# dernasherbrezon/sdr-server

Hardware: AMD Instinct MI355X
Metric: input IQ Msamples/s processed (all clients), 2.016 Msps->48 kHz xlating FIR (higher is better)
Workload: dtype f32; 1 GPU; 1024 clients x 48 kHz off one 2.016 Msps cu8 stream, D=42, 505 taps, 262144-byte blocks (BASELINE configs[3]; N=1: the >=1000-client single-GPU target); clients_total=1024, clients_per_gpu=1024, blocks_per_call=8, mode=optimized, parallelism=single GPU, rccl_ranks=1, feed=xlating_multi (C host)

## Files before the change

### sdr-server_amd/csrc/xl_kernels.hip

```cpp
#include "xl_dev_inline.h"

#include <hip/hip_ext.h>

#include <stdlib.h>

__global__ __launch_bounds__(64) void xl_nco_table_kernel(const XlNcoClient *__restrict__ cl, uint32_t n,
                                                          const float2 *state_in, float2 *state_out,
                                                          float2 *__restrict__ tab, const XlPos pos,
                                                          const uint32_t explicit_K, const uint32_t prio,
                                                          const uint32_t lanes) {
  if (prio == 3) __builtin_amdgcn_s_setprio(3);
  else if (prio == 2) __builtin_amdgcn_s_setprio(2);
  else if (prio == 1) __builtin_amdgcn_s_setprio(1);
  if (threadIdx.x >= lanes) return;
  const uint32_t c = blockIdx.x * lanes + threadIdx.x;
  if (c >= n) return;
  const XlNcoClient k = cl[c];
  const XlBnd bnd = xl_nco_bnd(k, pos, explicit_K);
  asm volatile("" ::: "v255", "a255");
  xl_nco_client_chain<true>(k, bnd, 0u, bnd.K, state_in, state_out, tab);
}

#define XLC_RING 64u
XL_DEV uint32_t xl_lds_off(const void *p) { return (uint32_t)(uintptr_t)(__attribute__((address_space(3))) const char *)p; }
XL_DEV void xl_lds_post(const uint32_t addr, const uint32_t v) { asm volatile("ds_write_b32 %0, %1" ::"v"(addr), "v"(v) : "memory"); }
XL_DEV void xl_lds_post64(const uint32_t addr, const v2f v) { asm volatile("ds_write_b64 %0, %1" ::"v"(addr), "v"(v) : "memory"); }
XL_DEV uint32_t xl_lds_poll(const uint32_t addr) {
  uint32_t v;
  asm volatile("ds_read_b32 %0, %1\n\ts_waitcnt lgkmcnt(0)" : "=v"(v) : "v"(addr) : "memory");
  return v;
}

#define XLC_ALIGN ".p2align 6\n\t"
#define XLC_MUL "v_pk_mul_f32 %[t1], %[p], %[inc] op_sel_hi:[1,0]\n\tv_pk_mul_f32 %[t2], %[p], %[inc] op_sel:[0,1] op_sel_hi:[1,1]\n\t"
#define XLC_ADD "v_pk_add_f32 %[p], %[t1], %[t2] op_sel:[0,1] op_sel_hi:[1,0] neg_lo:[0,1]\n\t"
#define XLC_STEP XLC_MUL XLC_ADD
#define XLC_ENTRY                                                       \
  XLC_MUL "ds_write_b64 %[addr], %[p]\n\t" XLC_ADD                      \
  XLC_MUL "v_add_u32 %[cnt], 1, %[cnt]\n\t" XLC_ADD                     \
  XLC_MUL "ds_write_b32 %[paddr], %[cnt]\n\t" XLC_ADD                   \
  XLC_MUL "v_add_u32 %[off], 0x200, %[off]\n\t" XLC_ADD                 \
  XLC_MUL "v_and_b32 %[off], 0x7fff, %[off]\n\t" XLC_ADD                \
  XLC_MUL "v_add_u32 %[addr], %[off], %[base]\n\t" XLC_ADD              \
  XLC_STEP XLC_STEP XLC_STEP XLC_STEP XLC_STEP XLC_STEP XLC_STEP XLC_STEP XLC_STEP XLC_STEP
#define XLC_STEPS10 XLC_STEP XLC_STEP XLC_STEP XLC_STEP XLC_STEP XLC_STEP XLC_STEP XLC_STEP XLC_STEP XLC_STEP
#define XLC_QENTRY(OFFS) XLC_MUL "ds_write_b64 %[addr], %[p] offset:" OFFS "\n\t" XLC_ADD XLC_STEP XLC_STEP
#define XLC_BLOCK_END(N, ADV)                                           \
  XLC_MUL "v_add_u32 %[cnt], " N ", %[cnt]\n\t" XLC_ADD                 \
  XLC_MUL "ds_write_b32 %[paddr], %[cnt]\n\t" XLC_ADD                   \
  XLC_MUL "v_add_u32 %[off], " ADV ", %[off]\n\t" XLC_ADD               \
  XLC_MUL "v_and_b32 %[off], 0x7fff, %[off]\n\t" XLC_ADD                \
  XLC_MUL "v_add_u32 %[addr], %[off], %[base]\n\t" XLC_ADD XLC_STEP XLC_STEP XLC_STEP XLC_STEP XLC_STEP XLC_STEP XLC_STEP XLC_STEP XLC_STEP XLC_STEP
#define XLC_QUAD                                                        \
  XLC_QENTRY("0") XLC_STEP XLC_STEP XLC_STEP XLC_STEPS10                \
  XLC_QENTRY("512") XLC_STEP XLC_STEP XLC_STEP XLC_STEPS10              \
  XLC_QENTRY("1024") XLC_STEP XLC_STEP XLC_STEP XLC_STEPS10             \
  XLC_MUL "ds_write_b64 %[addr], %[p] offset:1536\n\t" XLC_ADD XLC_BLOCK_END("4", "0x800")
#define XLC_E(OFFS) XLC_QENTRY(OFFS) XLC_STEP XLC_STEP XLC_STEP XLC_STEPS10
#define XLC_E7(B0, B1, B2, B3, B4, B5, B6) XLC_E(B0) XLC_E(B1) XLC_E(B2) XLC_E(B3) XLC_E(B4) XLC_E(B5) XLC_E(B6)
#define XLC_E8(B0, B1, B2, B3, B4, B5, B6, B7) XLC_E7(B0, B1, B2, B3, B4, B5, B6) XLC_E(B7)
#define XLC_OCT                                                         \
  XLC_E7("0", "512", "1024", "1536", "2048", "2560", "3072")           \
  XLC_MUL "ds_write_b64 %[addr], %[p] offset:3584\n\t" XLC_ADD XLC_BLOCK_END("8", "0x1000")
#define XLC_HEX                                                         \
  XLC_E8("0", "512", "1024", "1536", "2048", "2560", "3072", "3584")   \
  XLC_E7("4096", "4608", "5120", "5632", "6144", "6656", "7168")       \
  XLC_MUL "ds_write_b64 %[addr], %[p] offset:7680\n\t" XLC_ADD XLC_BLOCK_END("16", "0x2000")
#define XLC_B32                                                         \
  XLC_E8("0", "512", "1024", "1536", "2048", "2560", "3072", "3584")   \
  XLC_E8("4096", "4608", "5120", "5632", "6144", "6656", "7168", "7680") \
  XLC_E8("8192", "8704", "9216", "9728", "10240", "10752", "11264", "11776") \
  XLC_E7("12288", "12800", "13312", "13824", "14336", "14848", "15360") \
  XLC_MUL "ds_write_b64 %[addr], %[p] offset:15872\n\t" XLC_ADD XLC_BLOCK_END("32", "0x4000")
static_assert(XL_PH_STRIDE == 16u && XLC_RING * 64u * 8u == 0x8000u, "XLC_ENTRY is written for 16 steps per entry and a 32 KB ring");

__global__ __launch_bounds__(256) void xl_nco_chain_kernel(const XlNcoClient *__restrict__ cl, uint32_t n,
                                                           const float2 *state_in, const XlChainCalls calls,
                                                           XlPos pos, unsigned long long *stats) {
  asm volatile("" ::: "v255", "a255");
  const unsigned long long t_entry = stats ? wall_clock64() : 0ull;
  __shared__ v2f ring[XLC_RING][64];
  __shared__ uint32_t s_emax;
  __shared__ uint32_t s_prod;
  __shared__ uint32_t s_next[3];
  const uint32_t w = __builtin_amdgcn_readfirstlane(threadIdx.x >> 6), lane = threadIdx.x & 63u;
  const uint32_t c = blockIdx.x * 64u + lane;
  const bool have = c < n;
  XlNcoClient k;
  k.incr = make_float2(1.0f, 0.0f);
  k.out_off = 0u, k.slot = 0u, k.D = 1u, k.rem0 = 0u;
  if (have) k = cl[c];
  v2f p = {1.0f, 0.0f};
  if (w == 0 && have) p = (v2f){state_in[k.slot].x, state_in[k.slot].y};
  unsigned long long cyc = 0ull, ticks = 0ull, wfirst = 0ull;
  uint32_t entries = 0u;
  for (uint32_t call = 0; call < calls.n; ++call, pos = xl_grid_next(pos)) {
    float2 *const tab = calls.tab[call];
    float2 *const state_out = calls.state_out[call];
    if (call) __syncthreads();
    XlBnd bnd = xl_nco_bnd(k, pos, 0xFFFFFFFFu);
    if (!have) bnd.K = 0u;
    const uint32_t K = bnd.K, E = (K + XL_PH_STRIDE - 1u) >> XL_PH_SHIFT;
    if (threadIdx.x == 0) {
      s_emax = 0u;
      s_prod = 0u;
      s_next[0] = 0u, s_next[1] = 1u, s_next[2] = 2u;
    }
    __syncthreads();
    if (w == 0 && E > 0u) atomicMax(&s_emax, E);
    __syncthreads();
    const uint32_t Emax = s_emax;
    const uint32_t a_prod = xl_lds_off(&s_prod), a_ring0 = xl_lds_off(&ring[0][0]), a_ring = xl_lds_off(&ring[0][lane]);
    v2f *__restrict__ o = reinterpret_cast<v2f *>(tab) + (k.out_off >> XL_PH_SHIFT);
    if (w == 0) {
      __builtin_amdgcn_s_setprio(3);
      const v2f inc = {k.incr.x, k.incr.y};
      uint32_t nb = xl_bnd_next(bnd, 0u);
      const uint32_t a_n0 = xl_lds_off(&s_next[0]), a_n1 = xl_lds_off(&s_next[1]), a_n2 = xl_lds_off(&s_next[2]);
      const unsigned long long c0 = stats ? clock64() : 0ull, w0 = stats ? wall_clock64() : 0ull;
      uint32_t e = 0;
      while (e < Emax) {
        uint32_t ev = (e << XL_PH_SHIFT) < K ? (nb < K ? nb : K) : 0xFFFFFFFFu;
#pragma unroll
        for (int sh = 1; sh < 64; sh <<= 1) {
          const uint32_t other = (uint32_t)__shfl_xor((int)ev, sh);
          ev = other < ev ? other : ev;
        }
        const uint32_t evs = __builtin_amdgcn_readfirstlane(ev);
        uint32_t e_stop = evs == 0u ? 0u : (evs - 1u) >> XL_PH_SHIFT;
        e_stop = e_stop < Emax ? e_stop : Emax;
        if (pos.pad & XL_POS_FMA_STEP) e_stop = e;
        if ((e << XL_PH_SHIFT) < K) {
          uint32_t ee = e;
          while (ee < e_stop) {
            if ((ee & (XLC_RING / 2u - 1u)) == 0u && ee >= XLC_RING) {
              const uint32_t q = (ee - XLC_RING / 2u) >> 1;
              for (uint32_t spin = 0; spin < (1u << 22); ++spin) {
                if (xl_lds_poll(a_n0) >= q && xl_lds_poll(a_n1) >= q && xl_lds_poll(a_n2) >= q) break;
                __builtin_amdgcn_s_sleep(1);
              }
            }
            const uint32_t next_check = (ee | (XLC_RING / 2u - 1u)) + 1u;
            const uint32_t chunk_end = e_stop < next_check ? e_stop : next_check;
            uint32_t off = ((ee & (XLC_RING - 1u)) << 9) + lane * (uint32_t)sizeof(v2f);
            uint32_t addr = a_ring0 + off, cnt = ee;
            v2f t1, t2;
#define XLC_RUN(BLOCK)                                                                                            \
  asm volatile(XLC_ALIGN BLOCK                                                                                   \
               : [p] "+v"(p), [off] "+v"(off), [addr] "+v"(addr), [cnt] "+v"(cnt), [t1] "=&v"(t1), [t2] "=&v"(t2) \
               : [inc] "v"(inc), [base] "v"(a_ring0), [paddr] "v"(a_prod)                                        \
               : "memory")
            for (; ee < chunk_end && (ee & 3u) != 0u; ++ee) XLC_RUN(XLC_ENTRY);
            if ((ee & 7u) == 4u && ee + 4u <= chunk_end) {
              XLC_RUN(XLC_QUAD);
              ee += 4u;
            }
            if ((ee & 15u) == 8u && ee + 8u <= chunk_end) {
              XLC_RUN(XLC_OCT);
              ee += 8u;
            }
            if ((ee & 31u) == 16u && ee + 16u <= chunk_end) {
              XLC_RUN(XLC_HEX);
              ee += 16u;
            }
            for (; ee + 32u <= chunk_end; ee += 32u) XLC_RUN(XLC_B32);
            for (; ee + 16u <= chunk_end; ee += 16u) XLC_RUN(XLC_HEX);
            for (; ee + 8u <= chunk_end; ee += 8u) XLC_RUN(XLC_OCT);
            for (; ee + 4u <= chunk_end; ee += 4u) XLC_RUN(XLC_QUAD);
            for (; ee < chunk_end; ++ee) XLC_RUN(XLC_ENTRY);
#undef XLC_RUN
          }
        }
        if (e_stop > e) e = e_stop;
        if (e < Emax) {
          if ((e & (XLC_RING / 2u - 1u)) == 0u && e >= XLC_RING) {
            const uint32_t q = (e - XLC_RING / 2u) >> 1;
            for (uint32_t spin = 0; spin < (1u << 22); ++spin) {
              if (xl_lds_poll(a_n0) >= q && xl_lds_poll(a_n1) >= q && xl_lds_poll(a_n2) >= q) break;
              __builtin_amdgcn_s_sleep(1);
            }
          }
          const uint32_t m0 = e << XL_PH_SHIFT;
          if (m0 < K) xl_lds_post64(a_ring + (e & (XLC_RING - 1u)) * 64u * (uint32_t)sizeof(v2f), p);
          xl_lds_post(a_prod, e + 1u);
          for (uint32_t m = m0; m < m0 + XL_PH_STRIDE && m < K; ++m) {
            p = xl_nco_next_any(p, inc, bnd.flags);
            if (m + 1u == nb) {
              p = xl_nco_renorm(p);
              nb = xl_bnd_next(bnd, m + 1u);
            }
          }
          ++e;
        }
      }
      if (have) state_out[k.slot] = make_float2(p.x, p.y);
      if (stats) {
        cyc += clock64() - c0;
        const unsigned long long w1 = wall_clock64();
        ticks += w1 - w0;
        entries += Emax;
        if (call == 0u) wfirst = w0;
        if (lane == 0u && blockIdx.x < 1024u) {
          stats[8192u + 8u * blockIdx.x + 1u + 2u * call] = w0 - t_entry;
          stats[8192u + 8u * blockIdx.x + 2u + 2u * call] = w1 - t_entry;
        }
      }
      continue;
    }
    const uint32_t j = w - 1u;
    const uint32_t a_next = xl_lds_off(&s_next[j]);
    v4f *__restrict__ o4 = reinterpret_cast<v4f *>(o);
    for (uint32_t q = j; 2u * q < Emax; q += 3u) {
      const uint32_t need = 2u * q + 2u < Emax ? 2u * q + 2u : Emax;
      for (uint32_t spin = 0; spin < (1u << 24); ++spin) {
        if (xl_lds_poll(a_prod) >= need) break;
        __builtin_amdgcn_s_sleep(1);
      }
      if (2u * q < E) {
        v2f a, b2 = {0.0f, 0.0f};
        const uint32_t ra = a_ring + ((2u * q) & (XLC_RING - 1u)) * 64u * (uint32_t)sizeof(v2f);
        const uint32_t rb = a_ring + ((2u * q + 1u) & (XLC_RING - 1u)) * 64u * (uint32_t)sizeof(v2f);
        const bool two = 2u * q + 1u < E;
        asm volatile("ds_read_b64 %0, %1" : "=v"(a) : "v"(ra) : "memory");
        if (two) asm volatile("ds_read_b64 %0, %1" : "=v"(b2) : "v"(rb) : "memory");
        asm volatile("s_waitcnt lgkmcnt(0)" ::: "memory");
        if (two) o4[q] = (v4f){a.x, a.y, b2.x, b2.y};
        else o[2u * q] = a;
      }
      xl_lds_post(a_next, q + 3u);
    }
    xl_lds_post(a_next, 0xFFFFFFFFu);
  }
  if (stats) __syncthreads();
  if (stats && threadIdx.x == 0u) {
    if (blockIdx.x < 1024u) {
      stats[8192u + 8u * blockIdx.x] = t_entry;
      stats[8192u + 8u * blockIdx.x + 7u] = wall_clock64() - t_entry;
    }
    stats[4u * blockIdx.x] = cyc;
    stats[4u * blockIdx.x + 1u] = ticks;
    stats[4u * blockIdx.x + 2u] = entries;
    stats[4u * blockIdx.x + 3u] = wfirst;
  }
}

template <int FMT>
XL_DEV void xl_stage_window(const XlFirArgs &a, const uint32_t zero_below, const uint32_t win0, const uint32_t wlen,
                            v2f *__restrict__ win) {
  const uint32_t bd = blockDim.x;
  for (uint32_t j0 = threadIdx.x; j0 < wlen; j0 += 4u * bd) {
    v2f v[4];
    bool ok[4];
#pragma unroll
    for (int u = 0; u < 4; ++u) {
      const uint32_t j = j0 + u * bd;
      const uint32_t s = win0 + j;
      const bool first = s < a.n0;
      ok[u] = j < wlen && s >= zero_below && (first || s - a.n0 < a.n1);
      const void *src = (first || !ok[u]) ? a.in0 : a.in1;
      const uint32_t idx = ok[u] ? (first ? s : s - a.n0) : 0u;
      v[u] = xl_sample(src, FMT, idx);
    }
#pragma unroll
    for (int u = 0; u < 4; ++u) {
      const uint32_t j = j0 + u * bd;
      if (j < wlen) win[j] = ok[u] ? v[u] : (v2f){0.0f, 0.0f};
    }
  }
}

template <int CT, int MODE, bool WIDE>
__global__ __launch_bounds__(64 * XL_NW_MAX) __attribute__((amdgpu_num_sgpr(96))) void xl_fir_kernel(const XlFirArgs a) {
  extern __shared__ __attribute__((aligned(16))) v2f xl_win[];
  const uint32_t OT = a.ota;

  if (blockIdx.x < a.nco_blocks) {
    if (((a.flags >> 4) & 3u) == 3u) __builtin_amdgcn_s_setprio(3);
    else if (((a.flags >> 4) & 3u) == 2u) __builtin_amdgcn_s_setprio(2);
    else if (((a.flags >> 4) & 3u) == 1u) __builtin_amdgcn_s_setprio(1);
    const uint32_t nwave = threadIdx.x >> 6, nlane = threadIdx.x & 63u;
    if (nwave < a.nco_wpw && nlane < XL_NCO_LANES) {
      const unsigned long long t0 = a.trace ? wall_clock64() : 0ull;
      const uint32_t c = (blockIdx.x * a.nco_wpw + nwave) * XL_NCO_LANES + nlane;
      if (c < a.nco_nclients) {
        const XlNcoClient k = a.nco_clients[c];
        const XlBnd bnd = xl_nco_bnd(k, xl_grid_next(a.pos), 0xFFFFFFFFu);
        xl_nco_client_chain<false>(k, bnd, 0u, bnd.K, a.nco_state_in, a.nco_state_out, a.nco_tab);
      }
      if (a.trace && nlane == 0) {
        unsigned long long *tn = a.trace + ((size_t)blockIdx.x * XL_NW_MAX + nwave) * 6;
        tn[0] = t0;
        tn[3] = wall_clock64();
        tn[4] = __builtin_amdgcn_s_getreg((4 << 0) | (0 << 6) | (31 << 11));
        tn[5] = __builtin_amdgcn_s_getreg((20 << 0) | (0 << 6) | (31 << 11));
      }
    }
    return;
  }

  if (!(a.flags & 2u)) __builtin_amdgcn_s_setprio(3);
  const uint32_t b = blockIdx.x - a.nco_blocks;
  const unsigned long long t_entry = a.trace ? wall_clock64() : 0ull;

  const uint32_t roll_blocks = gridDim.x - a.nco_blocks < XL_ROLL_BLOCKS ? gridDim.x - a.nco_blocks : XL_ROLL_BLOCKS;
  if (a.hist_out != nullptr && b < roll_blocks) {
    const uint16_t *__restrict__ h0 = reinterpret_cast<const uint16_t *>(a.in0);
    const uint16_t *__restrict__ h1 = reinterpret_cast<const uint16_t *>(a.in1);
    uint16_t *__restrict__ ho = reinterpret_cast<uint16_t *>(a.hist_out);
    const uint32_t hu = a.hist_units, nu = a.block_units;
    for (uint32_t j = b * blockDim.x + threadIdx.x; j < hu; j += roll_blocks * blockDim.x) {
      const uint32_t sidx = nu + j;
      ho[j] = (sidx < hu) ? h0[sidx] : h1[sidx - hu];
    }
  }
  const uint32_t xcd = b & 7u, idx = b >> 3;
  const uint32_t total = a.ngroups * a.xtiles;
  const uint32_t per = total >> 3, extra = total & 7u;
  const uint32_t len = per + (xcd < extra ? 1u : 0u);
  if (idx >= len) return;
  const uint32_t wi = xcd * per + (xcd < extra ? xcd : extra) + idx;
  const uint32_t y = wi / a.xtiles;
  const uint32_t x = wi - y * a.xtiles;
  if (y >= a.ngroups) return;

  const cu32_p g = (cu32_p)(uintptr_t)(a.groups + y);
  const uint32_t D = g[0], Tpad = g[2], ntiles = g[4];
  const XlDyn d = a.explicit_dyn ? a.dyn1 : xl_grid_dyn(D, g[1], g[3], g[7], a.pos);
  const uint32_t K = d.K;
  const bool live = x * OT < K;
  if (!live && a.nco_lanes == 0u) return;

  const uint32_t w = __builtin_amdgcn_readfirstlane(threadIdx.x >> 6);
  v2f phs[CT];
#pragma unroll
  for (int c = 0; c < CT; ++c) phs[c] = (v2f){1.0f, 0.0f};
  if (live) {
    if (w < ntiles) {
      constexpr uint32_t G = 64u / XL_PH_STRIDE;
      const uint32_t lane = threadIdx.x & 63u;
      v2f *__restrict__ pl = xl_win + w * (CT * 64u);
      const uint32_t *__restrict__ tg = reinterpret_cast<const uint32_t *>(a.groups + y) + 8u + w * XL_TILE_DWORDS;
      const uint32_t c = lane / G, e = lane % G;
      const uint32_t m0 = x * OT + e * XL_PH_STRIDE;
      if (c < tg[1] && e * XL_PH_STRIDE < OT && m0 < K) {
        const uint32_t off = tg[2 + c];
        const float2 ci = reinterpret_cast<const float2 *>(tg + 2 + XL_CT_MAX)[c];
        const uint32_t left = K - m0, span = OT < XL_PH_STRIDE ? OT : XL_PH_STRIDE;
        XlBnd bnd;
        bnd.j0 = d.j0, bnd.D = D, bnd.S = a.pos.S, bnd.G = a.explicit_dyn ? 1u : a.pos.G, bnd.K = K, bnd.flags = a.pos.pad;
        v2f *__restrict__ dst = pl + c * 64u + e * XL_PH_STRIDE;
        xl_phase_walk((reinterpret_cast<const v2f *>(a.phtab) + (off >> XL_PH_SHIFT))[m0 >> XL_PH_SHIFT], m0,
                      left < span ? left : span, (v2f){ci.x, ci.y}, bnd, [&](uint32_t i, v2f ph) { dst[i] = ph; });
      }
      __builtin_amdgcn_wave_barrier();
#pragma unroll
      for (int cc = 0; cc < CT; ++cc) phs[cc] = pl[cc * 64u + lane];
    }
    __syncthreads();

    const uint32_t win0 = d.base + x * OT * D;
    const uint32_t wlen = (OT - 1u) * D + Tpad;
    if (a.fmt == XLF_CU8) xl_stage_window<XLF_CU8>(a, d.zero_below, win0, wlen, xl_win);
    else if (a.fmt == XLF_CS8) xl_stage_window<XLF_CS8>(a, d.zero_below, win0, wlen, xl_win);
    else if (a.fmt == XLF_CS16) xl_stage_window<XLF_CS16>(a, d.zero_below, win0, wlen, xl_win);
    else xl_stage_window<XLF_CF32>(a, d.zero_below, win0, wlen, xl_win);
  }
  __syncthreads();

  if (w >= ntiles) {
    const uint32_t nlane = threadIdx.x & 63u;
    const uint32_t slot = (g[6] + (w - ntiles)) * a.xtiles + x;
    if (a.nco_lanes != 0u && slot < a.nco_slots && nlane < a.nco_lanes) {
      __builtin_amdgcn_s_setprio(3);
      const unsigned long long t0 = a.trace ? wall_clock64() : 0ull;
      const uint32_t c = slot * a.nco_lanes + nlane;
      if (c < a.nco_nclients) {
        const XlNcoClient k = a.nco_clients[c];
        const XlBnd bnd = xl_nco_bnd(k, xl_grid_next(a.pos), 0xFFFFFFFFu);
        xl_nco_client_chain<false>(k, bnd, 0u, bnd.K, a.nco_state_in, a.nco_state_out, a.nco_tab);
      }
      if (a.trace && nlane == 0) {
        unsigned long long *tn = a.trace + ((size_t)blockIdx.x * XL_NW_MAX + w) * 6;
        tn[0] = t0;
        tn[3] = wall_clock64();
        tn[4] = __builtin_amdgcn_s_getreg((4 << 0) | (0 << 6) | (31 << 11));
        tn[5] = __builtin_amdgcn_s_getreg((20 << 0) | (0 << 6) | (31 << 11));
      }
    }
    return;
  }
  if (!live) return;
  const uint32_t lane = threadIdx.x & 63u;
  unsigned long long *tr = a.trace ? a.trace + ((size_t)blockIdx.x * XL_NW_MAX + w) * 6 : nullptr;
  if (tr && lane == 0) {
    tr[0] = t_entry;
    tr[1] = wall_clock64();
    tr[4] = __builtin_amdgcn_s_getreg((4 << 0) | (0 << 6) | (31 << 11));
    tr[5] = __builtin_amdgcn_s_getreg((20 << 0) | (0 << 6) | (31 << 11));
  }
  const cu32_p t = g + 8 + w * XL_TILE_DWORDS;
  const uint32_t ncl = t[1];
  const cfloat_p tp = (cfloat_p)(uintptr_t)(a.taps + t[0]);

  XlAcc<MODE> acc[CT];
#pragma unroll
  for (int c = 0; c < CT; ++c) acc[c].clear();

  constexpr int STEP = (CT == 9 || CT == 10) ? 6 : 4;
  const v2f *lp = xl_win + (lane >= OT ? 0u : lane) * D;
#define XL_TAP_LOOP(I0, I1)                                                                       \
  for (uint32_t i = (I0); i < (I1); i += STEP) {                                                  \
    v2f xs[STEP];                                                                                 \
    if (WIDE) {                                                                                   \
      _Pragma("unroll") for (int u = 0; u < STEP; u += 2) {                                       \
        const v4f q = *reinterpret_cast<const v4f *>(lp + i + u);                                 \
        xs[u] = (v2f){q.x, q.y};                                                                  \
        xs[u + 1] = (v2f){q.z, q.w};                                                              \
      }                                                                                           \
    } else {                                                                                      \
      _Pragma("unroll") for (int u = 0; u < STEP; ++u) xs[u] = lp[i + u];                         \
    }                                                                                             \
    const cfloat_p tq = tp + (size_t)i * (2 * CT);                                                \
    _Pragma("unroll") for (int u = 0; u < STEP; ++u) {                                            \
      _Pragma("unroll") for (int c = 0; c < CT; ++c)                                              \
        acc[c].mac(xs[u], tq[(u * CT + c) * 2], tq[(u * CT + c) * 2 + 1]);                        \
    }                                                                                             \
  }
  if (a.flags & 2u) {
    XL_TAP_LOOP(0u, Tpad)
  } else {
    const uint32_t steps = Tpad / STEP;
    const uint32_t b1 = steps / 2, b2 = (7 * steps) / 8;
    const uint32_t e1 = b1 * STEP < Tpad ? b1 * STEP : Tpad;
    const uint32_t e2 = b2 * STEP < Tpad ? b2 * STEP : Tpad;
    __builtin_amdgcn_s_setprio(2);
    XL_TAP_LOOP(0u, e1)
    __builtin_amdgcn_s_setprio(1);
    XL_TAP_LOOP(e1, e2)
    __builtin_amdgcn_s_setprio(0);
    XL_TAP_LOOP(e2, Tpad)
    __builtin_amdgcn_s_setprio(3);
  }
#undef XL_TAP_LOOP

  if (tr && lane == 0) tr[2] = wall_clock64();
  v2f *__restrict__ out = reinterpret_cast<v2f *>(a.out);
  {
    const uint32_t m = x * OT + lane;
    if (m < K && lane < OT) {
#pragma unroll
      for (int c = 0; c < CT; ++c) {
        if ((uint32_t)c < ncl) out[t[2 + c] + m] = xl_rotate<MODE>(acc[c].value(), phs[c]);
      }
    }
  }
  if (tr && lane == 0) {
    __builtin_amdgcn_s_waitcnt(0);
    tr[3] = wall_clock64();
  }
}

size_t xl_fir_lds_bytes_ota(uint32_t D, uint32_t Tpad, uint32_t ota) {
  return ((size_t)(ota - 1u) * D + Tpad) * sizeof(v2f);
}

uint32_t xl_fir_pick_ota(uint32_t D, uint32_t Tpad, size_t budget) {
  for (uint32_t ota = 64; ota >= 8; ota >>= 1)
    if (xl_fir_lds_bytes_ota(D, Tpad, ota) <= budget) return ota;
  return 0;
}

template <int CT, int MODE, bool WIDE>
static hipError_t xl_fir_go2(int nw, const XlFirArgs &a, size_t lds, hipStream_t s) {
  static bool attr_done = false;
  if (!attr_done) {
    hipError_t e = hipFuncSetAttribute(reinterpret_cast<const void *>(&xl_fir_kernel<CT, MODE, WIDE>),
                                       hipFuncAttributeMaxDynamicSharedMemorySize, 160 * 1024);
    if (e != hipSuccess) return e;
    attr_done = true;
  }
  const uint32_t nblocks = a.nco_blocks + 8u * ((a.ngroups * a.xtiles + 7u) / 8u);
  if (nblocks == 0) return hipSuccess;
  const size_t need = (size_t)nw * CT * 64u * sizeof(float2);
  if (lds < need) lds = need;
  hipLaunchKernelGGL((xl_fir_kernel<CT, MODE, WIDE>), dim3(nblocks), dim3(64 * nw), lds, s, a);
  return hipGetLastError();
}

template <int CT, int MODE>
static hipError_t xl_fir_go(int nw, const XlFirArgs &a, size_t lds, hipStream_t s) {
  return (a.flags & 1u) ? xl_fir_go2<CT, MODE, true>(nw, a, lds, s) : xl_fir_go2<CT, MODE, false>(nw, a, lds, s);
}

hipError_t xl_launch_fir(int ct, int mode, int nw, const XlFirArgs &a, size_t lds, hipStream_t s) {
  if (lds > 160 * 1024 || nw < 1 || nw > XL_NW_MAX) return hipErrorInvalidValue;
  if (a.ota != 64 && a.ota != 32 && a.ota != 16 && a.ota != 8) return hipErrorInvalidValue;
  switch (ct * 2 + (mode ? 1 : 0)) {
    case 2: return xl_fir_go<1, 0>(nw, a, lds, s);
    case 3: return xl_fir_go<1, 1>(nw, a, lds, s);
    case 4: return xl_fir_go<2, 0>(nw, a, lds, s);
    case 5: return xl_fir_go<2, 1>(nw, a, lds, s);
    case 8: return xl_fir_go<4, 0>(nw, a, lds, s);
    case 9: return xl_fir_go<4, 1>(nw, a, lds, s);
    case 16: return xl_fir_go<8, 0>(nw, a, lds, s);
    case 17: return xl_fir_go<8, 1>(nw, a, lds, s);
    case 18: return xl_fir_go<9, 0>(nw, a, lds, s);
    case 19: return xl_fir_go<9, 1>(nw, a, lds, s);
    case 20: return xl_fir_go<10, 0>(nw, a, lds, s);
    case 21: return xl_fir_go<10, 1>(nw, a, lds, s);
    case 24: return xl_fir_go<12, 0>(nw, a, lds, s);
    case 25: return xl_fir_go<12, 1>(nw, a, lds, s);
    default: return hipErrorInvalidValue;
  }
}

hipError_t xl_launch_nco_table(const XlNcoClient *clients, uint32_t nclients, const float2 *state_in,
                               float2 *state_out, float2 *phtab, XlPos pos, uint32_t explicit_K, uint32_t prio,
                               hipStream_t s) {
  if (nclients == 0) return hipSuccess;
  const uint32_t lanes = XL_NCO_LANES;
  hipLaunchKernelGGL(xl_nco_table_kernel, dim3((nclients + lanes - 1) / lanes), dim3(64), 0, s, clients, nclients,
                     state_in, state_out, phtab, pos, explicit_K, prio, lanes);
  return hipGetLastError();
}

hipError_t xl_launch_nco_chain(const XlNcoClient *clients, uint32_t nclients, const float2 *state_in,
                               const XlChainCalls &calls, XlPos pos, unsigned long long *stats, hipStream_t s,
                               hipEvent_t done) {
  if (calls.n < 1u || calls.n > XL_CHAIN_MAXCALLS) return hipErrorInvalidValue;
  if (nclients == 0) return done ? hipEventRecord(done, s) : hipSuccess;
  if (done)
    hipExtLaunchKernelGGL(xl_nco_chain_kernel, dim3((nclients + 63u) / 64u), dim3(256), 0, s, nullptr, done, 0, clients,
                          nclients, state_in, calls, pos, stats);
  else
    hipLaunchKernelGGL(xl_nco_chain_kernel, dim3((nclients + 63u) / 64u), dim3(256), 0, s, clients, nclients, state_in,
                       calls, pos, stats);
  return hipGetLastError();
}

__global__ void xl_convert_cf32_kernel(const void *__restrict__ raw, int fmt, uint32_t n, v2f *__restrict__ dst) {
  for (uint32_t i = blockIdx.x * blockDim.x + threadIdx.x; i < n; i += gridDim.x * blockDim.x)
    dst[i] = xl_sample(raw, fmt, i);
}

hipError_t xl_launch_convert_cf32(const void *raw, int fmt, uint32_t nsamples, float2 *dst, hipStream_t s) {
  if (nsamples == 0) return hipSuccess;
  const uint32_t blocks = (nsamples + 255) / 256 < 2048 ? (nsamples + 255) / 256 : 2048;
  hipLaunchKernelGGL(xl_convert_cf32_kernel, dim3(blocks), dim3(256), 0, s, raw, fmt, nsamples,
                     reinterpret_cast<v2f *>(dst));
  return hipGetLastError();
}

__global__ void xl_convert_q15_kernel(const void *__restrict__ raw, int fmt, uint32_t n, int16_t *__restrict__ dst) {
  for (uint32_t i = blockIdx.x * blockDim.x + threadIdx.x; i < n; i += gridDim.x * blockDim.x) {
    int32_t v;
    if (fmt == XLF_CU8) {
      v = ((int32_t) reinterpret_cast<const uint8_t *>(raw)[i] - 128) * 256;
    } else if (fmt == XLF_CS8) {
      v = (int32_t) reinterpret_cast<const int8_t *>(raw)[i] * 256;
    } else {
      v = reinterpret_cast<const int16_t *>(raw)[i];
    }
    dst[i] = (int16_t)v;
  }
}

hipError_t xl_launch_convert_q15(const void *raw, int fmt, uint32_t nelems, int16_t *dst, hipStream_t s) {
  if (nelems == 0) return hipSuccess;
  const uint32_t blocks = (nelems + 255) / 256 < 2048 ? (nelems + 255) / 256 : 2048;
  hipLaunchKernelGGL(xl_convert_q15_kernel, dim3(blocks), dim3(256), 0, s, raw, fmt, nelems, dst);
  return hipGetLastError();
}

__global__ __launch_bounds__(1024) void xl_move_down_kernel(uint32_t *buf, uint32_t from_dw, uint32_t count_dw) {
  for (uint32_t base = 0; base < count_dw; base += 1024) {
    const uint32_t i = base + threadIdx.x;
    uint32_t v = 0;
    if (i < count_dw) v = buf[from_dw + i];
    __syncthreads();
    if (i < count_dw) buf[i] = v;
    __syncthreads();
  }
}

hipError_t xl_launch_move_down(void *buf, uint32_t from, uint32_t count, uint32_t elem_bytes, hipStream_t s) {
  if (count == 0 || from == 0) return hipSuccess;
  const uint32_t k = elem_bytes / 4;
  hipLaunchKernelGGL(xl_move_down_kernel, dim3(1), dim3(1024), 0, s, reinterpret_cast<uint32_t *>(buf), from * k,
                     count * k);
  return hipGetLastError();
}

__global__ void xl_update_history_kernel(const uint16_t *__restrict__ hist, const uint16_t *__restrict__ block,
                                         uint32_t h_u, uint32_t n_u, uint16_t *__restrict__ out) {
  for (uint32_t j = blockIdx.x * blockDim.x + threadIdx.x; j < h_u; j += gridDim.x * blockDim.x) {
    const uint32_t s = n_u + j;
    out[j] = (s < h_u) ? hist[s] : block[s - h_u];
  }
}

hipError_t xl_launch_update_history(const void *hist, const void *block, uint32_t h, uint32_t n, uint32_t bps,
                                    void *new_hist, hipStream_t s) {
  if (h == 0) return hipSuccess;
  const uint32_t u = bps / 2;
  const uint32_t hu = h * u, nu = n * u;
  const uint32_t blocks = (hu + 255) / 256 < 256 ? (hu + 255) / 256 : 256;
  hipLaunchKernelGGL(xl_update_history_kernel, dim3(blocks), dim3(256), 0, s, reinterpret_cast<const uint16_t *>(hist),
                     reinterpret_cast<const uint16_t *>(block), hu, nu, reinterpret_cast<uint16_t *>(new_hist));
  return hipGetLastError();
}


XL_DEV uint32_t xl_q15_step(const uint32_t p, const uint32_t a, const uint32_t b) {
  typedef short s2 __attribute__((ext_vector_type(2)));
  const int32_t tr = __builtin_amdgcn_sdot2(__builtin_bit_cast(s2, p), __builtin_bit_cast(s2, a), 0, false);
  const int32_t ti = __builtin_amdgcn_sdot2(__builtin_bit_cast(s2, p), __builtin_bit_cast(s2, b), 0, false);
  return __builtin_bit_cast(uint32_t, __builtin_amdgcn_cvt_pk_i16(tr >> 15, ti >> 15));
}

__global__ void xl_nco_table_q15_kernel(int32_t ir, int32_t ii, const short2 *state_in, short2 *state_out,
                                        uint32_t *__restrict__ tab, uint32_t K) {
  if (blockIdx.x != 0 || threadIdx.x != 0) return;
  const uint32_t a = ((uint32_t)ir & 0xFFFFu) | ((uint32_t)(-ii) << 16), b = ((uint32_t)ii & 0xFFFFu) | ((uint32_t)ir << 16);
  uint32_t p = ((uint32_t)(uint16_t)state_in->x) | ((uint32_t)(uint16_t)state_in->y << 16);
  uint32_t m = 0;
  for (; m + XL_PH_STRIDE <= K; m += XL_PH_STRIDE) {
    tab[m >> XL_PH_SHIFT] = p;
#pragma unroll
    for (uint32_t i = 0; i < XL_PH_STRIDE; ++i) p = xl_q15_step(p, a, b);
  }
  if (m < K) tab[m >> XL_PH_SHIFT] = p;
  for (; m < K; ++m) p = xl_q15_step(p, a, b);
  *state_out = make_short2((short)(p & 0xFFFFu), (short)(p >> 16));
}

hipError_t xl_launch_nco_table_q15(int16_t incr_re, int16_t incr_im, const short2 *state_in, short2 *state_out, short2 *phtab,
                                   uint32_t K, hipStream_t s) {
  if (K == 0) return hipSuccess;
  hipLaunchKernelGGL(xl_nco_table_q15_kernel, dim3(1), dim3(64), 0, s, (int32_t)incr_re, (int32_t)incr_im, state_in, state_out,
                     reinterpret_cast<uint32_t *>(phtab), K);
  return hipGetLastError();
}

__global__ __launch_bounds__(256) void xl_fir_q15_kernel(const uint32_t *__restrict__ work, const uint32_t *taps,
                                                         uint32_t T, uint32_t D, uint32_t K, int32_t ir, int32_t ii,
                                                         const uint32_t *__restrict__ phtab, short2 *__restrict__ out) {
  typedef short s2 __attribute__((ext_vector_type(2)));
  const uint32_t m = blockIdx.x * blockDim.x + threadIdx.x;
  if (m >= K) return;
  const uint32_t *__restrict__ w = work + (size_t)m * D;
  const cu32_p tq = (cu32_p)(uintptr_t)taps;
  long long sr = 0, si = 0;
  auto mac = [&](const uint32_t xv, const uint32_t hv) {
    const int32_t hr = (int16_t)(hv & 0xFFFFu), hi = (int32_t)hv >> 16;
    const int32_t xr = (int16_t)(xv & 0xFFFFu), xi = (int32_t)xv >> 16;
    const uint32_t swp = (hv >> 16) | (hv << 16);
    si += (long long)__builtin_amdgcn_sdot2(__builtin_bit_cast(s2, xv), __builtin_bit_cast(s2, swp), 0, false);
    sr += (long long)(xr * hr - xi * hi);
  };
  uint32_t i = 0;
  if ((((uintptr_t)w) & 7u) == 0u) {
    for (; i + 2u <= T; i += 2u) {
      const uint2 xv = *reinterpret_cast<const uint2 *>(w + i);
      mac(xv.x, tq[i]);
      mac(xv.y, tq[i + 1u]);
    }
  }
  for (; i < T; ++i) mac(w[i], tq[i]);
  const int32_t ar = xl_sat16((int32_t)(sr >> 15));
  const int32_t ai = xl_sat16((int32_t)(si >> 15));
  const uint32_t a = ((uint32_t)ir & 0xFFFFu) | ((uint32_t)(-ii) << 16), b = ((uint32_t)ii & 0xFFFFu) | ((uint32_t)ir << 16);
  uint32_t p = phtab[m >> XL_PH_SHIFT];
  for (uint32_t k = m & (XL_PH_STRIDE - 1u); k > 0u; --k) p = xl_q15_step(p, a, b);
  const int32_t pr = (int16_t)(p & 0xFFFFu), pi = (int32_t)p >> 16;
  const int32_t tr = ar * pr - ai * pi;
  const int32_t ti = ar * pi + ai * pr;
  out[m] = make_short2((short)xl_sat16(tr >> 15), (short)xl_sat16(ti >> 15));
}

hipError_t xl_launch_fir_q15(const short2 *work, const short2 *taps, uint32_t T, uint32_t D, uint32_t K, int16_t incr_re,
                             int16_t incr_im, const short2 *phtab, short2 *out, hipStream_t s) {
  if (K == 0) return hipSuccess;
  hipLaunchKernelGGL(xl_fir_q15_kernel, dim3((K + 63) / 64), dim3(64), 0, s, reinterpret_cast<const uint32_t *>(work),
                     reinterpret_cast<const uint32_t *>(taps), T, D, K, (int32_t)incr_re, (int32_t)incr_im,
                     reinterpret_cast<const uint32_t *>(phtab), out);
  return hipGetLastError();
}


__global__ __launch_bounds__(64) void xl_nco_q15_batch_kernel(const XlNcoClient *__restrict__ cl, const uint32_t *__restrict__ qinc,
                                                              uint32_t n, short2 *qstate, short2 *__restrict__ tab, const XlPos pos) {
  const uint32_t c = blockIdx.x * 64u + threadIdx.x;
  if (c >= n) return;
  const XlNcoClient k = cl[c];
  const uint32_t K = xl_nco_bnd(k, pos, 0xFFFFFFFFu).K;
  const int32_t ir = (int16_t)(qinc[c] & 0xFFFFu), ii = (int16_t)(qinc[c] >> 16);
  int32_t pr = qstate[k.slot].x, pi = qstate[k.slot].y;
  short2 *__restrict__ o = tab + (k.out_off >> XL_PH_SHIFT);
  for (uint32_t m = 0; m < K; ++m) {
    if ((m & (XL_PH_STRIDE - 1u)) == 0u) o[m >> XL_PH_SHIFT] = make_short2((short)pr, (short)pi);
    const int32_t tr = pr * ir - pi * ii, ti = pr * ii + pi * ir;
    pr = xl_sat16(tr >> 15);
    pi = xl_sat16(ti >> 15);
  }
  qstate[k.slot] = make_short2((short)pr, (short)pi);
}

hipError_t xl_launch_nco_q15_batch(const XlNcoClient *clients, const uint32_t *qinc, uint32_t nclients, short2 *qstate,
                                   short2 *qphtab, XlPos pos, hipStream_t s) {
  if (nclients == 0) return hipSuccess;
  hipLaunchKernelGGL(xl_nco_q15_batch_kernel, dim3((nclients + 63u) / 64u), dim3(64), 0, s, clients, qinc, nclients, qstate,
                     qphtab, pos);
  return hipGetLastError();
}

typedef const double __attribute__((address_space(4))) *cdouble_p;

template <int CT>
__global__ __launch_bounds__(64 * XL_NW_MAX) void xl_fir_q15_batch_kernel(const XlFirArgs a, const double *__restrict__ qtaps,
                                                                          const short2 *__restrict__ qphtab) {
  extern __shared__ __attribute__((aligned(16))) v2f xl_qwin[];
  const uint32_t OT = a.ota;
  const uint32_t b = blockIdx.x;
  const uint32_t roll_blocks = gridDim.x < XL_ROLL_BLOCKS ? gridDim.x : XL_ROLL_BLOCKS;
  if (a.hist_out != nullptr && b < roll_blocks) {
    const uint16_t *__restrict__ h0 = reinterpret_cast<const uint16_t *>(a.in0);
    const uint16_t *__restrict__ h1 = reinterpret_cast<const uint16_t *>(a.in1);
    uint16_t *__restrict__ ho = reinterpret_cast<uint16_t *>(a.hist_out);
    for (uint32_t j = b * blockDim.x + threadIdx.x; j < a.hist_units; j += roll_blocks * blockDim.x) {
      const uint32_t sidx = a.block_units + j;
      ho[j] = (sidx < a.hist_units) ? h0[sidx] : h1[sidx - a.hist_units];
    }
  }
  const uint32_t y = b / a.xtiles, x = b - y * a.xtiles;
  if (y >= a.ngroups) return;
  const cu32_p g = (cu32_p)(uintptr_t)(a.groups + y);
  const uint32_t D = g[0], T = g[1], Tpad = g[2], ntiles = g[4];
  const XlDyn d = xl_grid_dyn(D, T, g[3], g[7], a.pos);
  const uint32_t K = d.K;
  if (x * OT >= K) return;
  {
    const uint32_t win0 = d.base + x * OT * D, wlen = (OT - 1u) * D + Tpad;
    for (uint32_t j = threadIdx.x; j < wlen; j += blockDim.x) {
      const uint32_t sidx = win0 + j;
      const bool first = sidx < a.n0;
      const bool ok = sidx >= d.zero_below && (first || sidx - a.n0 < a.n1);
      const v2f v = xl_sample_q15((first || !ok) ? a.in0 : a.in1, a.fmt, ok ? (first ? sidx : sidx - a.n0) : 0u);
      xl_qwin[j] = ok ? v : (v2f){0.0f, 0.0f};
    }
  }
  __syncthreads();
  const uint32_t w = __builtin_amdgcn_readfirstlane(threadIdx.x >> 6), lane = threadIdx.x & 63u;
  if (w >= ntiles) return;
  const cu32_p t = g + 8 + w * XL_TILE_DWORDS;
  const uint32_t ncl = t[1];
  const cdouble_p tq = (cdouble_p)(uintptr_t)(qtaps + (size_t)t[0] * 2u);
  double accr[CT], acci[CT];
#pragma unroll
  for (int c = 0; c < CT; ++c) accr[c] = acci[c] = 0.0;
  const v2f *lp = xl_qwin + (lane >= OT ? 0u : lane) * D;
  for (uint32_t i = 0; i < T; ++i) {
    const v2f xs = lp[i];
    const double xr = (double)xs.x, xi = (double)xs.y;
    const cdouble_p h = tq + (size_t)i * (2 * CT);
#pragma unroll
    for (int c = 0; c < CT; ++c) {
      const double hr = h[2 * c], hi = h[2 * c + 1];
      accr[c] = __builtin_fma(xr, hr, accr[c]);
      accr[c] = __builtin_fma(-xi, hi, accr[c]);
      acci[c] = __builtin_fma(xr, hi, acci[c]);
      acci[c] = __builtin_fma(xi, hr, acci[c]);
    }
  }
  const uint32_t m = x * OT + lane;
  if (m >= K || lane >= OT) return;
#pragma unroll
  for (int c = 0; c < CT; ++c) {
    if ((uint32_t)c >= ncl) continue;
    const uint32_t off = t[2 + c], qi = t[2 + 3 * XL_CT_MAX + c];
    const int32_t ar = xl_sat16((int32_t)__builtin_floor(accr[c] * (1.0 / 32768.0)));
    const int32_t ai = xl_sat16((int32_t)__builtin_floor(acci[c] * (1.0 / 32768.0)));
    const short2 p0 = qphtab[(off >> XL_PH_SHIFT) + (m >> XL_PH_SHIFT)];
    const int32_t ir = (int16_t)(qi & 0xFFFFu), ii = (int16_t)(qi >> 16);
    int32_t pr = p0.x, pi = p0.y;
    for (uint32_t j = m & (XL_PH_STRIDE - 1u); j > 0u; --j) {
      const int32_t tr = pr * ir - pi * ii, ti = pr * ii + pi * ir;
      pr = xl_sat16(tr >> 15);
      pi = xl_sat16(ti >> 15);
    }
    const int32_t orr = ar * pr - ai * pi, oi = ar * pi + ai * pr;
    reinterpret_cast<short2 *>(a.out + off)[m] = make_short2((short)xl_sat16(orr >> 15), (short)xl_sat16(oi >> 15));
  }
}

template <int CT>
static hipError_t xl_fir_q15_go(int nw, const XlFirArgs &a, const double *qtaps, const short2 *qphtab, size_t lds, hipStream_t s) {
  static bool attr_done = false;
  if (!attr_done) {
    hipError_t e = hipFuncSetAttribute(reinterpret_cast<const void *>(&xl_fir_q15_batch_kernel<CT>),
                                       hipFuncAttributeMaxDynamicSharedMemorySize, 160 * 1024);
    if (e != hipSuccess) return e;
    attr_done = true;
  }
  const uint32_t nblocks = a.ngroups * a.xtiles;
  if (nblocks == 0) return hipSuccess;
  hipLaunchKernelGGL((xl_fir_q15_batch_kernel<CT>), dim3(nblocks), dim3(64 * nw), lds, s, a, qtaps, qphtab);
  return hipGetLastError();
}

hipError_t xl_launch_fir_q15_batch(int ct, int nw, const XlFirArgs &a, const double *qtaps, const short2 *qphtab,
                                   size_t lds, hipStream_t s) {
  if (lds > 160 * 1024 || nw < 1 || nw > XL_NW_MAX) return hipErrorInvalidValue;
  switch (ct) {
    case 1: return xl_fir_q15_go<1>(nw, a, qtaps, qphtab, lds, s);
    case 2: return xl_fir_q15_go<2>(nw, a, qtaps, qphtab, lds, s);
    case 4: return xl_fir_q15_go<4>(nw, a, qtaps, qphtab, lds, s);
    case 8: return xl_fir_q15_go<8>(nw, a, qtaps, qphtab, lds, s);
    case 9: return xl_fir_q15_go<9>(nw, a, qtaps, qphtab, lds, s);
    case 10: return xl_fir_q15_go<10>(nw, a, qtaps, qphtab, lds, s);
    case 12: return xl_fir_q15_go<12>(nw, a, qtaps, qphtab, lds, s);
    default: return hipErrorInvalidValue;
  }
}
```

Baseline: 5.567 million Msamples/s.

## Fold consumer-drain polling into the B32 NCO loop and cache a ring credit limit

The producer wavefront now keeps a cached limit of ring entries it may write, derived from the consumers' progress counters. It polls and sleeps only when that limit would be exceeded, instead of polling every half ring. The 32-entry block becomes a self-looping inline-asm loop that reads the three consumer counters mid-block and continues while room remains. The event-boundary reduction now takes a ballot fast path when all lanes agree. Per-block cycle stats are also added. This cuts spin and branch overhead on the serial NCO chain, at the cost of hand-scheduled asm with scalar-register hazards and s_nop padding that must be correct.

Result: faster. 5.674 million Msamples/s, median of 6 (+1.9%).

```diff
diff --git a/sdr-server_amd/csrc/xl_kernels.hip b/sdr-server_amd/csrc/xl_kernels.hip
--- a/sdr-server_amd/csrc/xl_kernels.hip
+++ b/sdr-server_amd/csrc/xl_kernels.hip
@@ -29,6 +29,38 @@
   uint32_t v;
   asm volatile("ds_read_b32 %0, %1\n\ts_waitcnt lgkmcnt(0)" : "=v"(v) : "v"(addr) : "memory");
   return v;
+}
+
+XL_DEV uint32_t xl_lds_poll3_min(const uint32_t a0, const uint32_t a1, const uint32_t a2) {
+  uint32_t v0, v1, v2;
+  asm volatile("ds_read_b32 %0, %3\n\tds_read_b32 %1, %4\n\tds_read_b32 %2, %5\n\ts_waitcnt lgkmcnt(0)"
+               : "=&v"(v0), "=&v"(v1), "=&v"(v2)
+               : "v"(a0), "v"(a1), "v"(a2)
+               : "memory");
+  v0 = v0 < v1 ? v0 : v1;
+  return v0 < v2 ? v0 : v2;
+}
+XL_DEV uint32_t xl_chain_lim(const uint32_t mn) { return mn >= 0x7FFFFFE0u ? 0xFFFFFFFFu : 2u * mn + XLC_RING; }
+XL_DEV uint32_t xl_chain_wait_drained(const uint32_t upto, const uint32_t a0, const uint32_t a1, const uint32_t a2) {
+  uint32_t lim = 0u;
+  for (uint32_t spin = 0; spin < (1u << 22); ++spin) {
+    lim = xl_chain_lim((uint32_t)__builtin_amdgcn_readfirstlane((int)xl_lds_poll3_min(a0, a1, a2)));
+    if (upto <= lim) break;
+    __builtin_amdgcn_s_sleep(1);
+  }
+  return lim;
+}
+XL_DEV uint32_t xl_chain_event(uint32_t ev) {
+  const unsigned long long act = __ballot(ev != 0xFFFFFFFFu);
+  if (act == 0ull) return 0xFFFFFFFFu;
+  const uint32_t first = (uint32_t)__builtin_amdgcn_readlane((int)ev, (int)__ffsll((long long)act) - 1);
+  if (__ballot(ev != 0xFFFFFFFFu && ev != first) == 0ull) return first;
+#pragma unroll
+  for (int sh = 1; sh < 64; sh <<= 1) {
+    const uint32_t other = (uint32_t)__shfl_xor((int)ev, sh);
+    ev = other < ev ? other : ev;
+  }
+  return (uint32_t)__builtin_amdgcn_readfirstlane((int)ev);
 }
 
 #define XLC_ALIGN ".p2align 6\n\t"
@@ -66,12 +98,27 @@
   XLC_E8("0", "512", "1024", "1536", "2048", "2560", "3072", "3584")   \
   XLC_E7("4096", "4608", "5120", "5632", "6144", "6656", "7168")       \
   XLC_MUL "ds_write_b64 %[addr], %[p] offset:7680\n\t" XLC_ADD XLC_BLOCK_END("16", "0x2000")
-#define XLC_B32                                                         \
-  XLC_E8("0", "512", "1024", "1536", "2048", "2560", "3072", "3584")   \
-  XLC_E8("4096", "4608", "5120", "5632", "6144", "6656", "7168", "7680") \
-  XLC_E8("8192", "8704", "9216", "9728", "10240", "10752", "11264", "11776") \
-  XLC_E7("12288", "12800", "13312", "13824", "14336", "14848", "15360") \
-  XLC_MUL "ds_write_b64 %[addr], %[p] offset:15872\n\t" XLC_ADD XLC_BLOCK_END("32", "0x4000")
+#define XLC_STEP2(I1, I2) XLC_MUL I1 "\n\t" XLC_ADD I2 "\n\t"
+#define XLC_B32_LOOP                                                                                         \
+  XLC_E8("0", "512", "1024", "1536", "2048", "2560", "3072", "3584")                                       \
+  XLC_E8("4096", "4608", "5120", "5632", "6144", "6656", "7168", "7680")                                   \
+  XLC_E8("8192", "8704", "9216", "9728", "10240", "10752", "11264", "11776")                               \
+  XLC_E("12288") XLC_E("12800") XLC_E("13312") XLC_E("13824") XLC_E("14336") XLC_E("14848")               \
+  XLC_QENTRY("15360")                                                                                      \
+  XLC_MUL "ds_read_b32 %[mn], %[an0]\n\t" XLC_ADD                                                           \
+  XLC_MUL "ds_read_b32 %[n1], %[an1]\n\t" XLC_ADD                                                           \
+  XLC_MUL "ds_read_b32 %[n2], %[an2]\n\t" XLC_ADD XLC_STEPS10                                               \
+  XLC_MUL "ds_write_b64 %[addr], %[p] offset:15872\n\t" XLC_ADD                                             \
+  XLC_MUL "v_add_u32 %[cnt], 32, %[cnt]\n\t" XLC_ADD "s_sub_u32 %[todo], %[todo], 1\n\t"                    \
+  XLC_MUL "ds_write_b32 %[paddr], %[cnt]\n\t" XLC_ADD                                                       \
+  XLC_MUL "v_add_u32 %[off], 0x4000, %[off]\n\t" XLC_ADD                                                    \
+  XLC_MUL "v_and_b32 %[off], 0x7fff, %[off]\n\t" XLC_ADD                                                    \
+  XLC_STEP2("v_add_u32 %[addr], %[off], %[base]", "s_add_u32 %[need], %[need], 16")                         \
+  XLC_STEP2("s_waitcnt lgkmcnt(0)", "v_min_u32 %[mn], %[mn], %[n1]")                                        \
+  XLC_STEP2("v_min_u32 %[mn], %[mn], %[n2]", "s_nop 0")                                                     \
+  XLC_STEP2("v_readfirstlane_b32 %[sm], %[mn]", "s_nop 0")                                                  \
+  XLC_STEP2("s_cmp_ge_u32 %[sm], %[need]", "s_cselect_b32 %[st], %[todo], 0")                               \
+  XLC_STEP XLC_STEP XLC_STEP XLC_STEP XLC_STEP XLC_STEP
 static_assert(XL_PH_STRIDE == 16u && XLC_RING * 64u * 8u == 0x8000u, "XLC_ENTRY is written for 16 steps per entry and a 32 KB ring");
 
 __global__ __launch_bounds__(256) void xl_nco_chain_kernel(const XlNcoClient *__restrict__ cl, uint32_t n,
@@ -109,7 +156,7 @@
     __syncthreads();
     if (w == 0 && E > 0u) atomicMax(&s_emax, E);
     __syncthreads();
-    const uint32_t Emax = s_emax;
+    const uint32_t Emax = (uint32_t)__builtin_amdgcn_readfirstlane((int)s_emax);
     const uint32_t a_prod = xl_lds_off(&s_prod), a_ring0 = xl_lds_off(&ring[0][0]), a_ring = xl_lds_off(&ring[0][lane]);
     v2f *__restrict__ o = reinterpret_cast<v2f *>(tab) + (k.out_off >> XL_PH_SHIFT);
     if (w == 0) {
@@ -118,31 +165,28 @@
       uint32_t nb = xl_bnd_next(bnd, 0u);
       const uint32_t a_n0 = xl_lds_off(&s_next[0]), a_n1 = xl_lds_off(&s_next[1]), a_n2 = xl_lds_off(&s_next[2]);
       const unsigned long long c0 = stats ? clock64() : 0ull, w0 = stats ? wall_clock64() : 0ull;
+      unsigned long long t_region = 0ull, t_drain = 0ull, t_b32 = 0ull;
+      uint32_t n_drain = 0u, n_b32 = 0u, n_event = 0u, n_runs = 0u;
       uint32_t e = 0;
+      uint32_t lim = XLC_RING;
+      uint32_t evs = xl_chain_event(0u < K ? (nb < K ? nb : K) : 0xFFFFFFFFu);
       while (e < Emax) {
-        uint32_t ev = (e << XL_PH_SHIFT) < K ? (nb < K ? nb : K) : 0xFFFFFFFFu;
-#pragma unroll
-        for (int sh = 1; sh < 64; sh <<= 1) {
-          const uint32_t other = (uint32_t)__shfl_xor((int)ev, sh);
-          ev = other < ev ? other : ev;
-        }
-        const uint32_t evs = __builtin_amdgcn_readfirstlane(ev);
         uint32_t e_stop = evs == 0u ? 0u : (evs - 1u) >> XL_PH_SHIFT;
         e_stop = e_stop < Emax ? e_stop : Emax;
         if (pos.pad & XL_POS_FMA_STEP) e_stop = e;
+        const unsigned long long r0 = stats ? clock64() : 0ull;
         if ((e << XL_PH_SHIFT) < K) {
           uint32_t ee = e;
           while (ee < e_stop) {
-            if ((ee & (XLC_RING / 2u - 1u)) == 0u && ee >= XLC_RING) {
-              const uint32_t q = (ee - XLC_RING / 2u) >> 1;
-              for (uint32_t spin = 0; spin < (1u << 22); ++spin) {
-                if (xl_lds_poll(a_n0) >= q && xl_lds_poll(a_n1) >= q && xl_lds_poll(a_n2) >= q) break;
-                __builtin_amdgcn_s_sleep(1);
-              }
+            const uint32_t left = e_stop - ee, slot = ee & (XLC_RING - 1u), room = XLC_RING - slot;
+            const uint32_t fit = left < room ? left : room;
+            const uint32_t nn = fit >= 32u ? 32u : fit >= 16u ? 16u : fit >= 8u ? 8u : fit >= 4u ? 4u : 1u;
+            if (ee + nn > lim) {
+              const unsigned long long d0 = stats ? clock64() : 0ull;
+              lim = xl_chain_wait_drained(ee + nn, a_n0, a_n1, a_n2);
+              if (stats) t_drain += clock64() - d0, ++n_drain;
             }
-            const uint32_t next_check = (ee | (XLC_RING / 2u - 1u)) + 1u;
-            const uint32_t chunk_end = e_stop < next_check ? e_stop : next_check;
-            uint32_t off = ((ee & (XLC_RING - 1u)) << 9) + lane * (uint32_t)sizeof(v2f);
+            uint32_t off = (slot << 9) + lane * (uint32_t)sizeof(v2f);
             uint32_t addr = a_ring0 + off, cnt = ee;
             v2f t1, t2;
 #define XLC_RUN(BLOCK)                                                                                            \
@@ -150,36 +194,40 @@
                : [p] "+v"(p), [off] "+v"(off), [addr] "+v"(addr), [cnt] "+v"(cnt), [t1] "=&v"(t1), [t2] "=&v"(t2) \
                : [inc] "v"(inc), [base] "v"(a_ring0), [paddr] "v"(a_prod)                                        \
                : "memory")
-            for (; ee < chunk_end && (ee & 3u) != 0u; ++ee) XLC_RUN(XLC_ENTRY);
-            if ((ee & 7u) == 4u && ee + 4u <= chunk_end) {
+            if (nn == 32u) {
+              const uint32_t want = (slot & 31u) == 0u ? left >> 5 : 1u;
+              uint32_t todo = want, need = (ee >> 1) - 16u, mn, n1, n2, sm, st;
+              const unsigned long long b0 = stats ? clock64() : 0ull;
+              asm volatile(XLC_ALIGN "1:\n\t" XLC_B32_LOOP "s_cmp_lg_u32 %[st], 0\n\ts_cbranch_scc1 1b\n\t"
+                           : [p] "+v"(p), [off] "+v"(off), [addr] "+v"(addr), [cnt] "+v"(cnt), [t1] "=&v"(t1), [t2] "=&v"(t2),
+                             [mn] "=&v"(mn), [n1] "=&v"(n1), [n2] "=&v"(n2), [todo] "+s"(todo), [need] "+s"(need), [sm] "=&s"(sm),
+                             [st] "=&s"(st)
+                           : [inc] "v"(inc), [base] "v"(a_ring0), [paddr] "v"(a_prod), [an0] "v"(a_n0), [an1] "v"(a_n1), [an2] "v"(a_n2)
+                           : "memory", "scc");
+              const uint32_t ran = (want - todo) << 5;
+              if (stats) t_b32 += clock64() - b0, n_b32 += ran, ++n_runs;
+              lim = xl_chain_lim(sm);
+              ee += ran;
+            } else if (nn == 16u) {
+              XLC_RUN(XLC_HEX);
+              ee += 16u;
+            } else if (nn == 8u) {
+              XLC_RUN(XLC_OCT);
+              ee += 8u;
+            } else if (nn == 4u) {
               XLC_RUN(XLC_QUAD);
               ee += 4u;
+            } else {
+              XLC_RUN(XLC_ENTRY);
+              ee += 1u;
             }
-            if ((ee & 15u) == 8u && ee + 8u <= chunk_end) {
-              XLC_RUN(XLC_OCT);
-              ee += 8u;
-            }
-            if ((ee & 31u) == 16u && ee + 16u <= chunk_end) {
-              XLC_RUN(XLC_HEX);
-              ee += 16u;
-            }
-            for (; ee + 32u <= chunk_end; ee += 32u) XLC_RUN(XLC_B32);
-            for (; ee + 16u <= chunk_end; ee += 16u) XLC_RUN(XLC_HEX);
-            for (; ee + 8u <= chunk_end; ee += 8u) XLC_RUN(XLC_OCT);
-            for (; ee + 4u <= chunk_end; ee += 4u) XLC_RUN(XLC_QUAD);
-            for (; ee < chunk_end; ++ee) XLC_RUN(XLC_ENTRY);
 #undef XLC_RUN
           }
         }
         if (e_stop > e) e = e_stop;
+        if (stats) t_region += clock64() - r0, ++n_event;
         if (e < Emax) {
-          if ((e & (XLC_RING / 2u - 1u)) == 0u && e >= XLC_RING) {
-            const uint32_t q = (e - XLC_RING / 2u) >> 1;
-            for (uint32_t spin = 0; spin < (1u << 22); ++spin) {
-              if (xl_lds_poll(a_n0) >= q && xl_lds_poll(a_n1) >= q && xl_lds_poll(a_n2) >= q) break;
-              __builtin_amdgcn_s_sleep(1);
-            }
-          }
+          if (e + 1u > lim) lim = xl_chain_wait_drained(e + 1u, a_n0, a_n1, a_n2);
           const uint32_t m0 = e << XL_PH_SHIFT;
           if (m0 < K) xl_lds_post64(a_ring + (e & (XLC_RING - 1u)) * 64u * (uint32_t)sizeof(v2f), p);
           xl_lds_post(a_prod, e + 1u);
@@ -191,6 +239,7 @@
             }
           }
           ++e;
+          evs = xl_chain_event((e << XL_PH_SHIFT) < K ? (nb < K ? nb : K) : 0xFFFFFFFFu);
         }
       }
       if (have) state_out[k.slot] = make_float2(p.x, p.y);
@@ -203,6 +252,13 @@
         if (lane == 0u && blockIdx.x < 1024u) {
           stats[8192u + 8u * blockIdx.x + 1u + 2u * call] = w0 - t_entry;
           stats[8192u + 8u * blockIdx.x + 2u + 2u * call] = w1 - t_entry;
+        }
+        if (lane == 0u && blockIdx.x < 128u) {
+          unsigned long long *const sp = stats + 4096u + 32u * blockIdx.x + 8u * call;
+          const unsigned long long k0 = clock64(), k1 = clock64(), k2 = clock64(), k3 = clock64(), k4 = clock64();
+          (void)k1, (void)k2, (void)k3;
+          sp[0] = k0 - c0, sp[1] = t_region, sp[2] = t_drain, sp[3] = t_b32;
+          sp[4] = n_drain, sp[5] = n_b32, sp[6] = n_event | ((unsigned long long)n_runs << 32), sp[7] = (k4 - k0) / 4ull;
         }
       }
       continue;
```
